# lmb-freiburg/hand3d

Measured on NVIDIA H100. Metric: images/sec full pipeline 320x320, higher is better.
Workload: dtype bf16 hi/lo split x3 MMA passes, fp32 accumulate (fp32 parity, 1e-3)

## Files before the change

### hand3d_b200/_lib.py

```python
from __future__ import annotations

import ctypes as C
import os

HERE = os.path.dirname(os.path.abspath(__file__))
LIB_PATH = os.path.join(HERE, "libhand3d_b200.so")

OK, EINVAL, ENODEVICE, ECUDA, EWEIGHTS, EWORKSPACE = 0, -1, -2, -3, -4, -5
PREC_FP32_FFMA, PREC_BF16X3, PREC_FP16X3, PREC_FP16, PREC_BF16 = 0, 1, 2, 3, 4
PRECISIONS = {"fp32_ffma": 0, "bf16x3": 1, "fp16x3": 2, "fp16": 3, "bf16": 4, "fp16_f8c": 5}
VARIANTS = {"direct": 0, "bottleneck": 1, "proposed": 2, "local": 3, "local_w_xyz_loss": 3}

_p, _i, _i64, _f = C.c_void_p, C.c_int, C.c_int64, C.c_float

SIGNATURES = {
    "h3d_last_error": (C.c_char_p, []),
    "h3d_version": (_i, []),
    "h3d_device_available": (_i, []),
    "h3d_create": (_i, [C.POINTER(_p), _i]),
    "h3d_destroy": (_i, [_p]),
    "h3d_set_precision": (_i, [_p, _i]),
    "h3d_get_precision": (_i, [_p]),
    "h3d_set_tuning": (_i, [_p, C.c_char_p, _i]),
    "h3d_check_errors": (_i, [_p, C.POINTER(_i)]),
# ... 11 lines not shown
    "h3d_pipeline_forward": (_i, [_p, _p, _p, _i, _i, _i, _i, _p, _p, _p, _p, _p, _p, _p, _p, _p, _p, _p]),
    "h3d_pose2d_forward": (_i, [_p, _p, _i, _i, _i, _p, _p, _p]),
    "h3d_track_state_bytes": (_i64, [_i]),
    "h3d_track_step": (_i, [_p, _p, _p, _i, _i, _i, _i, _i, _f, _f, _p, _p, _p, _p, _p, _p, _p, _p]),
    "h3d_track_update": (_i, [_p, _p, _p, _p, _p, _i, _f, _f, _p, _p]),
    "h3d_conv2d_f32": (_i, [_p, _p, _p, _p, _p, _i, _i, _i, _i, _i, _i, _i, _i, _p]),
    "h3d_conv2d_tc": (_i, [_p, _p, _p, _p, _p, _i, _i, _i, _i, _i, _i, _i, _i, _p]),
    "h3d_conv2d_tc_strided": (_i, [_p, _p, _p, _p, _p, _i, _i, _i, _i, _i, _i, _i, _i, _i, _p]),
    "h3d_pack_conv_weights": (_i, [_p, _p, _p, _i, _i, _i, _i, C.POINTER(_p)]),
    "h3d_free_packed_conv": (_i, [_p, _p]),
    "h3d_conv2d_tc_packed": (_i, [_p, _p, _p, _p, _i, _i, _i, _i, _i, _p]),
    "h3d_conv2d_tc_dev": (_i, [_p, _p, _p, _p, _p, _i, _i, _i, _i, _i, _i, _i, _i, _i, _p]),
    "h3d_conv2d_tc_backward": (_i, [_p, _p, _p, _p, _p, _p, _p, _p, _i, _i, _i, _i, _i, _i, _i, _i, _i, _p]),
    "h3d_conv2d_layer_planes": (_i, [_p, _p, _i, _i, _i, _i, _p, _p, _i, _i, _i, _p, _i, _i, _i, _i, _p, _p, _p, _p, _i, _i, _p, _i, _i, _p]),
    "h3d_conv2d_tc_geometry": (_i, [_i, _i, _i, _i, _i, _i, C.POINTER(_i)]),
    "h3d_conv2d_wgrad_geometry": (_i, [_i, _i, _i, _i, _i, _i, C.POINTER(_i)]),
    "h3d_leaky_relu_f32": (_i, [_p, _p, _p, _i64, _p]),
    "h3d_maxpool2x2_f32": (_i, [_p, _p, _p, _i, _i, _i, _i, _p]),
    "h3d_maxpool2x2_backward_f32": (_i, [_p, _p, _p, _p, _i, _i, _i, _i, _p]),
    "h3d_fully_connected_f32": (_i, [_p, _p, _p, _p, _p, _i, _i, _i, _i, _p]),
    "h3d_resize_bilinear_tf1": (_i, [_p, _p, _p, _i, _i, _i, _i, _i, _i, _p]),
    "h3d_avgpool8": (_i, [_p, _p, _p, _i, _i, _i, _i, _p]),
    "h3d_seg_postprocess": (_i, [_p, _p, _i, _i, _i, _p, _p, _p, _p, _p, _p]),
    "h3d_calc_center_bb": (_i, [_p, _p, _i, _i, _i, _p, _p, _p, _p]),
    "h3d_crop_image_from_xy": (_i, [_p, _p, _p, _p, _p, _i, _i, _i, _i, _i, _p]),
    "h3d_detect_keypoints": (_i, [_p, _p, _i, _i, _i, _i, _p, _p]),
    "h3d_upsample_detect_keypoints": (_i, [_p, _p, _i, _i, _i, _i, _i, _p, _p, _p]),
    "h3d_pack_records": (_i, [_p, _p, _p, _p, _p, _i, _p, _p]),
    "h3d_gather_records_p2p": (_i, [_p, _p, _p, _p, _p, _i, _i, _p, _p, C.c_uint64, _i, _i, C.c_uint32, _i64, _p]),
    "h3d_decode_records": (_i, [_p, _i, _p, _i, _i, _p, _p, _p, _p, _p]),
# ... 72 lines not shown
```

### hand3d_b200/csrc/api.cu

```cuda
#include <array>
#include <cstdarg>
#include <cstring>
#include <functional>
#include <map>
#include <memory>
#include <string>
#include <vector>

#include "common.cuh"
#include "split_fmt.cuh"

namespace h3d {

static thread_local char g_err[1024] = "";
void set_error(const char* fmt, ...) {
    va_list ap;
    va_start(ap, fmt);
    vsnprintf(g_err, sizeof(g_err), fmt, ap);
    va_end(ap);
}
int cuda_fail(cudaError_t e, const char* what, const char* file, int line) {
    set_error("CUDA error %d (%s) at %s:%d: %s", (int)e, cudaGetErrorString(e), file, line, what);
    if (e == cudaErrorNoDevice || e == cudaErrorInsufficientDriver) return H3D_ENODEVICE;
    return H3D_ECUDA;
// ... 1458 lines not shown
        d.partial = wpart; d.dw = dw_hwio; d.err_flag = ctx->err_flag;
        if ((rc = launch_conv_wgrad(d, s))) return rc;
        ctx->launches += 3;
    }
    return H3D_OK;
}

int h3d_conv2d_tc_geometry(int B, int H, int W, int Cout, int pool, int precision, int* out) {
    H3D_REQUIRE(out && B > 0 && H > 0 && W > 0 && Cout > 0, "h3d_conv2d_tc_geometry: bad argument");
    H3D_REQUIRE(pool >= 0 && pool <= 2, "h3d_conv2d_tc_geometry: pool must be 0 (none), 1 (max-pool) or 2 (stride 2)");
    H3D_REQUIRE(precision >= H3D_PREC_BF16X3 && precision <= H3D_PREC_FP16_F8C, "h3d_conv2d_tc_geometry: precision must be a tensor-core mode");
    tc_conv_geometry(B, H, W, (int)align_up(Cout, 64), pool, passes_of(precision), out);
    return H3D_OK;
}

int h3d_conv2d_wgrad_geometry(int B, int H, int W, int ksize, int Cin, int Cout, int* out) {
    H3D_REQUIRE(out && B > 0 && H > 0 && W > 0 && Cin > 0 && Cout > 0, "h3d_conv2d_wgrad_geometry: bad argument");
    H3D_REQUIRE(ksize == 1 || ksize == 3 || ksize == 5 || ksize == 7, "h3d_conv2d_wgrad_geometry: ksize must be 1, 3, 5 or 7");
    conv_wgrad_geometry(B, H, W, ksize, (int)align_up(Cin, 64), (int)align_up(Cout, 64), out);
    return H3D_OK;
}

int h3d_conv2d_tc(h3d_ctx* ctx, const float* x, const float* host_w_hwio, const float* host_bias, float* y, int B, int H, int W,
                  int Cin, int Cout, int ksize, int leaky, int precision, void* stream) {
    return h3d_conv2d_tc_strided(ctx, x, host_w_hwio, host_bias, y, B, H, W, Cin, Cout, ksize, 1, leaky, precision, stream);
}

int h3d_conv2d_tc_strided(h3d_ctx* ctx, const float* x, const float* host_w_hwio, const float* host_bias, float* y, int B, int H, int W,
                          int Cin, int Cout, int ksize, int stride, int leaky, int precision, void* stream) {
    H3D_REQUIRE(ctx != nullptr, "ctx is NULL");
// ... 524 lines not shown
```

### hand3d_b200/csrc/common.cuh

```cuda
#pragma once
#include <cuda_runtime.h>
#include <cuda_bf16.h>
#include <cuda_fp16.h>
#include <stdint.h>
#include <stdio.h>
#include <algorithm>
#include <cmath>
#include <string>

#include "../../include/hand3d_b200.h"

namespace h3d {

void set_error(const char* fmt, ...);
int cuda_fail(cudaError_t e, const char* what, const char* file, int line);

#define H3D_CUDA(expr)                                                     \
    do {                                                                   \
        cudaError_t _e = (expr);                                           \
        if (_e != cudaSuccess) return h3d::cuda_fail(_e, #expr, __FILE__, __LINE__); \
    } while (0)

#define H3D_CHECK_LAUNCH() H3D_CUDA(cudaGetLastError())

// ... 167 lines not shown
    int Cout, Cout_pad;
    Split y;
    int Cy_total, cy_off;
    float* yf;
    int Cyf_total, cyf_off;
    int B, H, W, k, leaky;
    int passes;
    float corr_scale = 0.f;
    Half16 half;
    int pool = 0;
    int* err_flag = nullptr;
};
struct TcTuning {
    int bn = 0;
    int chunk_kb = 0;
    int no_side_stream = 0, no_pool_fusion = 0, lift_direct = 0;
    int c3_ffma = 0;
    int no_seg_fusion = 0;
    int fc_chain = 1;
    int pdl = 1;
};
TcTuning& tc_tuning();
int tc_set_tuning(const char* key, int value);
struct FcLayerDesc {
    Split x; int x_stride, in_features;
    Split w; const float* bias; int out_features, out_pad;
    const float* w_scale = nullptr;
    Split y; int y_stride;
    float* yf; int yf_stride;
    int leaky;
};
struct FcChainDesc { FcLayerDesc layer[4]; int num_layers = 0; };
struct FcChainPlan;
FcChainPlan* fc_chain_plan_create(const FcChainDesc* chains, int num_chains, int B, Half16 half, const float* can, const float* uxyz,
                                  unsigned int* counter, int* err_flag);
void fc_chain_plan_destroy(FcChainPlan* p);
int fc_chain_launch(const FcChainPlan* p, const float* hand_side, float* rot, float* out, cudaStream_t s);
TcConvPlan* tc_conv_plan_create(const TcConvDesc& d, int* rc = nullptr);
void tc_conv_plan_destroy(TcConvPlan* p);
int tc_conv_launch(const TcConvPlan* p, cudaStream_t s);
int64_t tc_conv_flops(const TcConvPlan* p);
int tc_num_sms();
void tc_conv_geometry(int B, int H, int W, int Cout_pad, int pool, int passes, int out[4]);

int launch_pack_conv_w(const float* w_hwio, const float* bias, Split out, float* bias_pad, float* w_scale, int k, int Cin, int Cout,
                       int Cin_pad, int Cout_pad, bool dgrad, Half16 half, cudaStream_t s);
int conv_grad_prep_blocks(int64_t pixels, int64_t* pixels_per_block);
int launch_conv_grad_prep(const float* dy, const float* y, Split out, float* db_part, int B, int H, int W, int Cout, int Cout_pad,
                          int stride, int leaky, cudaStream_t s);
int launch_bias_grad_reduce(const float* db_part, int nblk, int Cout, int Cout_pad, float* db, cudaStream_t s);
struct WgradDesc {
    Split x;
    Split dy;
    int B, H, W, Cin, Cout, Cin_pad, Cout_pad, k, passes;
    float* partial;
    float* dw;
    int* err_flag;
};
// ... 28 lines not shown
```

### hand3d_b200/csrc/conv_wgmma.cu

```cuda
#include <cuda.h>

#include <algorithm>
#include <cstdlib>
#include <cstring>
#include <vector>

#include "common.cuh"
#include "split_fmt.cuh"
#include "wgmma_common.cuh"

namespace h3d {

namespace {

constexpr int BM = 128;
constexpr int BK = 64;
constexpr int kThreads = 384;
constexpr int kConsumerThreads = 256;
constexpr int A_TILE_BYTES = BM * BK * 2;
constexpr int STG_COLS = 64;
constexpr int STG_PITCH = STG_COLS + 1;
constexpr int STG_BYTES = BM * STG_PITCH * 4;
constexpr int kSmemBudget = 227 * 1024 - 2048 - STG_BYTES;

__host__ __device__ constexpr int stage_bytes(int BN, int PASSES) { return (PASSES >= 3 ? 2 : 1) * (A_TILE_BYTES + BN * BK * 2); }
__host__ __device__ constexpr int num_stages(int BN, int PASSES) {
    return kSmemBudget / stage_bytes(BN, PASSES) > 8 ? 8 : kSmemBudget / stage_bytes(BN, PASSES);
}
__host__ __device__ constexpr int smem_bytes(int BN, int PASSES) { return num_stages(BN, PASSES) * stage_bytes(BN, PASSES) + STG_BYTES + 2048; }

struct TcParams {
    const float* bias;
    uint16_t* y_hi; uint16_t* y_lo; uint8_t* y_l8; uint8_t* y_h8; int Cy_total, cy_off;
    float corr_scale;
    float* yf; int Cyf_total, cyf_off;
    int B, H, W, k, pad, cin_chunks;
    int TW, TH, TB, tiles_w, tiles_h, n_tiles, num_tiles;
    int n_valid;
    int pool;
    int chunk_kb;
    int leaky;
    int* err_flag;
    const float* w_scale;
};

template <int PASSES, bool FP16, bool SMEM_SCALE = false>
__device__ __forceinline__ void epilogue_store32(const TcParams& p, const float* a, int64_t pix, int n, bool valid, const float* w_scale) {
    float f[32];
    const float4* bp = reinterpret_cast<const float4*>(p.bias + n);
#pragma unroll
    for (int q = 0; q < 8; ++q) {
        const float4 bv = __ldg(bp + q);
        if (PASSES == 4) {
            f[4 * q + 0] = fmaf(a[4 * q + 0], p.corr_scale, bv.x);
            f[4 * q + 1] = fmaf(a[4 * q + 1], p.corr_scale, bv.y);
// ... 185 lines not shown
        fence_regs<NR8>(acc8);
        if constexpr (PASSES == 4) {
#pragma unroll
            for (int i = 0; i < NR; ++i) acc[i] += acc8[i];
        }
        if (kb0 == 0) {
#pragma unroll
            for (int i = 0; i < NR; ++i) racc[i] = acc[i];
        } else {
#pragma unroll
            for (int i = 0; i < NR; ++i) racc[i] += acc[i];
        }
    }
}

template <int BN, int PASSES, bool FP16, class PixOf, bool SMEM_SCALE = false>
__device__ __forceinline__ void store_tile(const TcParams& p, const float* racc, float* stg, int ct, int n0, PixOf pix_of,
                                           const float* w_scale) {
    const int wg = ct >> 7, tt = ct & 127;
    const int r0 = wg * 64 + (tt >> 5) * 16 + ((tt & 31) >> 2);
    const int cq = 2 * (tt & 3);
    const int row = ct & 127, half = ct >> 7;
    int64_t pix; bool valid;
    pix_of(row, pix, valid);
#pragma unroll
    for (int rnd = 0; rnd < BN / STG_COLS; ++rnd) {
        named_bar_sync(1, kConsumerThreads);
#pragma unroll
        for (int j = 0; j < STG_COLS / 8; ++j) {
            const int jj = rnd * (STG_COLS / 8) + j, c = 8 * j + cq;
            stg[r0 * STG_PITCH + c] = racc[4 * jj];
            stg[r0 * STG_PITCH + c + 1] = racc[4 * jj + 1];
            stg[(r0 + 8) * STG_PITCH + c] = racc[4 * jj + 2];
            stg[(r0 + 8) * STG_PITCH + c + 1] = racc[4 * jj + 3];
        }
        named_bar_sync(1, kConsumerThreads);
        float f[32];
#pragma unroll
        for (int q = 0; q < 32; ++q) f[q] = stg[row * STG_PITCH + half * 32 + q];
        epilogue_store32<PASSES, FP16, SMEM_SCALE>(p, f, pix, n0 + rnd * STG_COLS + half * 32, valid, w_scale);
    }
}

constexpr int kProducerRegs = 40, kConsumerRegs = 232;

template <int BN, int PASSES, bool FP16>
__global__ void __launch_bounds__(kThreads, 1)
conv_tc_kernel(const __grid_constant__ CUtensorMap map_x_hi, const __grid_constant__ CUtensorMap map_x_lo,
               const __grid_constant__ CUtensorMap map_w_hi, const __grid_constant__ CUtensorMap map_w_lo,
               const __grid_constant__ CUtensorMap map_x_h8, const __grid_constant__ CUtensorMap map_w_l8, const TcParams p) {
    using C = RingCfg<BN, PASSES>;
    static_assert(PASSES != 4 || FP16, "fp8-correction mode uses an fp16 main plane");
    static_assert(smem_bytes(BN, PASSES) <= 227 * 1024, "conv_tc_kernel: shared memory budget");

    extern __shared__ __align__(1024) uint8_t smem_raw[];
    uint8_t* smem = reinterpret_cast<uint8_t*>((reinterpret_cast<uintptr_t>(smem_raw) + 1023) & ~(uintptr_t)1023);
    float* stg = reinterpret_cast<float*>(smem + C::STAGES * C::STAGE_BYTES);
    uint64_t* bars = reinterpret_cast<uint64_t*>(smem + C::STAGES * C::STAGE_BYTES + STG_BYTES);
    Ring ring{smem, bars, bars + C::STAGES, 0, 0};

    const int warp = threadIdx.x >> 5, lane = threadIdx.x & 31;
    const int wg = __shfl_sync(0xFFFFFFFFu, (int)threadIdx.x / 128, 0);
    const int kblocks = p.k * p.k * p.cin_chunks;

    if (threadIdx.x == 0) {
        prefetch_tmap(&map_x_hi); prefetch_tmap(&map_w_hi);
        if (PASSES >= 3) { prefetch_tmap(&map_x_lo); prefetch_tmap(&map_w_lo); }
        if (PASSES == 4) { prefetch_tmap(&map_x_h8); prefetch_tmap(&map_w_l8); }
        for (int s = 0; s < C::STAGES; ++s) { mbar_init(&ring.full[s], 1); mbar_init(&ring.empty[s], kConsumerThreads / 32); }
        asm volatile("fence.mbarrier_init.release.cluster;" ::: "memory");
    }
    __syncthreads();
    pdl_launch_dependents();
    pdl_wait();

    if (wg == 0) {
        setmaxnreg_dec<kProducerRegs>();
        if (warp == 0) {
            for (int tile = blockIdx.x; tile < p.num_tiles; tile += gridDim.x) {
                const int nt = tile % p.n_tiles, mt = tile / p.n_tiles;
                const int tw = mt % p.tiles_w, th = (mt / p.tiles_w) % p.tiles_h, tb = mt / (p.tiles_w * p.tiles_h);
                const int w0 = tw * p.TW - p.pad, h0 = th * p.TH - p.pad, b0 = tb * p.TB, n0 = nt * BN;
                int kcol = 0;
                for (int kh = 0; kh < p.k; ++kh)
                    for (int kw = 0; kw < p.k; ++kw)
                        for (int cc = 0; cc < p.cin_chunks; ++cc, kcol += BK)
                            produce_kblock<BN, PASSES>(ring, &map_x_hi, &map_x_lo, &map_x_h8, &map_w_hi, &map_w_lo, &map_w_l8, cc * BK,
                                                       w0 + kw, h0 + kh, b0, kcol, n0, p.err_flag);
            }
        }
    } else {
        setmaxnreg_inc<kConsumerRegs>();
        const int ct = threadIdx.x - 128;
        float racc[BN / 2];
        for (int tile = blockIdx.x; tile < p.num_tiles; tile += gridDim.x) {
            const int nt = tile % p.n_tiles, mt = tile / p.n_tiles;
            const int tw = mt % p.tiles_w, th = (mt / p.tiles_w) % p.tiles_h, tb = mt / (p.tiles_w * p.tiles_h);
            mma_tile<BN, PASSES, FP16>(ring, kblocks, p.chunk_kb, racc, ct >> 7, lane, p.err_flag);
            store_tile<BN, PASSES, FP16>(p, racc, stg, ct, nt * BN, [&](int row, int64_t& pix, bool& valid) {
                const int w_l = row % p.TW, h_l = (row / p.TW) % p.TH, b_l = row / (p.TW * p.TH);
                const int w = tw * p.TW + w_l, h = th * p.TH + h_l, b = tb * p.TB + b_l;
                valid = (w < p.W) && (h < p.H) && (b < p.B);
                pix = ((int64_t)b * p.H + h) * p.W + w;
                if (p.pool) {
                    const int par = p.pool == 2 ? 1 : 0;
                    valid = valid && ((w & 1) == par) && ((h & 1) == par);
                    pix = ((int64_t)b * (p.H >> 1) + (h >> 1)) * (p.W >> 1) + (w >> 1);
                }
            }, p.w_scale);
        }
    }
}

constexpr int C3_TW = 16, C3_TH = 8;
constexpr int C3T_THREADS = 256;
constexpr int C3T_B_BYTES = 128 * BK * 2;
constexpr int C3T_PW = C3_TW + 2, C3T_PH = C3_TH + 2;
constexpr int C3T_PATCH_FLOATS = C3T_PH * C3T_PW * 3;
constexpr int C3T_SMEM = C3T_B_BYTES + 2 * A_TILE_BYTES + STG_BYTES + C3T_PATCH_FLOATS * 4 + 64 * 4 + 1024 ;

template <bool FP16>
__global__ void __launch_bounds__(C3T_THREADS, 2)
conv_c3_tc_kernel(const float* __restrict__ x, const float* __restrict__ w, const TcParams p) {
// ... 263 lines not shown
        const int64_t tiles = (int64_t)ceil_div(W, c[0]) * ceil_div(H, c[1]) * ceil_div(B, c[2]);
        if (best < 0 || tiles < best) { best = tiles; *TW = c[0]; *TH = c[1]; *TB = c[2]; }
    }
}

template <int BN, int PASSES, bool FP16>
int launch_inst(const TcConvPlan* pl, cudaStream_t s);

}

struct TcConvPlan {
    int device = 0;
    TcConvDesc d;
    CUtensorMap map_x_hi, map_x_lo, map_w_hi, map_w_lo, map_x_h8, map_w_l8;
    TcParams p;
    int BN, grid;
};

constexpr int kMaxDevices = 64;
static int current_device() { int dev = 0; if (cudaGetDevice(&dev) != cudaSuccess) { cudaGetLastError(); dev = 0; } return dev; }
int tc_num_sms() {
    static int n[kMaxDevices] = {};
    const int dev = current_device() % kMaxDevices;
    if (!n[dev]) {
        int v = 0;
        if (cudaDeviceGetAttribute(&v, cudaDevAttrMultiProcessorCount, dev) != cudaSuccess || v <= 0) { cudaGetLastError(); v = 132; }
        n[dev] = v;
    }
    return n[dev];
}
template <typename K>
// ... 11 lines not shown
    cudaLaunchConfig_t cfg = {};
    cfg.gridDim = grid; cfg.blockDim = block; cfg.dynamicSmemBytes = smem; cfg.stream = s;
    cudaLaunchAttribute attr[1];
    attr[0].id = cudaLaunchAttributeProgrammaticStreamSerialization;
    attr[0].val.programmaticStreamSerializationAllowed = tc_tuning().pdl ? 1 : 0;
    cfg.attrs = attr; cfg.numAttrs = 1;
    return cudaLaunchKernelEx(&cfg, kernel, static_cast<KArgs>(args)...);
}

TcTuning& tc_tuning() {
    static TcTuning t = [] {
        TcTuning v;
        auto geti = [](const char* n, int d) { const char* e = getenv(n); return e ? atoi(e) : d; };
        v.bn = geti("H3D_TC_BN", 0);
        v.chunk_kb = geti("H3D_TC_CHUNK_KB", 0);
        v.no_side_stream = geti("H3D_NO_SIDE_STREAM", 0);
        v.no_pool_fusion = geti("H3D_NO_POOL_FUSION", 0);
        v.lift_direct = geti("H3D_LIFT_DIRECT", 0);
        v.c3_ffma = geti("H3D_C3_FFMA", 0);
        v.pdl = geti("H3D_PDL", 1);
        v.fc_chain = geti("H3D_FC_CHAIN", 1);
        v.no_seg_fusion = geti("H3D_NO_SEG_FUSION", 0);
        return v;
    }();
    return t;
}
int tc_set_tuning(const char* key, int value) {
    TcTuning& t = tc_tuning();
    const std::string k(key ? key : "");
    if (k == "tc_bn") t.bn = value;
    else if (k == "tc_chunk_kb") t.chunk_kb = value;
    else if (k == "no_side_stream") t.no_side_stream = value;
    else if (k == "no_pool_fusion") t.no_pool_fusion = value;
    else if (k == "lift_direct") t.lift_direct = value;
    else if (k == "c3_ffma") t.c3_ffma = value;
    else if (k == "pdl") t.pdl = value;
    else if (k == "fc_chain") t.fc_chain = value;
    else if (k == "no_seg_fusion") t.no_seg_fusion = value;
    else { set_error("h3d_set_tuning: unknown key '%s'", k.c_str()); return H3D_EINVAL; }
    return H3D_OK;
}

namespace {
int choose_bn(int H, int W, int Cout_pad, int passes) {
    const TcTuning& tune = tc_tuning();
    int BN = Cout_pad % 128 == 0 ? 128 : 64;
    if ((int64_t)H * W <= 256) BN = 64;
    if ((tune.bn == 64 || tune.bn == 128) && Cout_pad % tune.bn == 0) BN = tune.bn;
    if (passes == 4) BN = 64;
    return BN;
}

template <int BN, int PASSES, bool FP16>
int launch_inst(const TcConvPlan* pl, cudaStream_t s) {
    constexpr int smem = smem_bytes(BN, PASSES);
    static bool attr[kMaxDevices] = {};
    if (int rc = smem_opt_in(conv_tc_kernel<BN, PASSES, FP16>, smem, attr)) return rc;
    H3D_CUDA(launch_pdl(conv_tc_kernel<BN, PASSES, FP16>, dim3(pl->grid), dim3(kThreads), smem, s, pl->map_x_hi, pl->map_x_lo, pl->map_w_hi,
                        pl->map_w_lo, pl->map_x_h8, pl->map_w_l8, pl->p));
    return H3D_OK;
}
}

TcConvPlan* tc_conv_plan_create(const TcConvDesc& d, int* rc) {
    int rc_local;
    if (!rc) rc = &rc_local;
    *rc = H3D_EINVAL;
    if (d.Cin_pad % BK != 0 || d.Cout_pad % 64 != 0 || (d.k != 1 && d.k != 3 && d.k != 5 && d.k != 7) || (d.passes != 1 && d.passes != 3 && d.passes != 4)) {
        set_error("tc_conv: unsupported geometry (Cin_pad=%d Cout_pad=%d k=%d passes=%d)", d.Cin_pad, d.Cout_pad, d.k, d.passes);
        return nullptr;
    }
    const bool padded_out = d.Cout % 32 != 0;
    if (d.y.hi && ((d.Cy_total % 8) || (d.cy_off % 8))) { set_error("tc_conv: split output channel offset/stride must be multiples of 8"); return nullptr; }
    if (d.yf && !padded_out && ((d.Cyf_total % 4) || (d.cyf_off % 4))) { set_error("tc_conv: fp32 output channel offset/stride must be multiples of 4"); return nullptr; }
// ... 23 lines not shown
    p.y_hi = d.y.hi; p.y_lo = d.y.lo; p.y_l8 = d.y.l8; p.y_h8 = d.y.h8; p.Cy_total = d.Cy_total; p.cy_off = d.cy_off;
    p.corr_scale = d.corr_scale;
    p.yf = d.yf; p.Cyf_total = d.Cyf_total; p.cyf_off = d.cyf_off;
    p.B = d.B; p.H = d.H; p.W = d.W; p.k = d.k; p.pad = d.k / 2; p.cin_chunks = d.Cin_pad / BK;
    p.TW = TW; p.TH = TH; p.TB = TB;
    p.tiles_w = ceil_div(d.W, TW); p.tiles_h = ceil_div(d.H, TH);
    p.n_tiles = d.Cout_pad / BN;
    p.num_tiles = p.tiles_w * p.tiles_h * ceil_div(d.B, TB) * p.n_tiles;
    p.leaky = d.leaky;
    p.n_valid = d.Cout;
    p.pool = d.pool;
    p.err_flag = d.err_flag;
    p.w_scale = d.w_scale;
    p.chunk_kb = d.passes >= 3 ? 9 : 27;
    if (tune.chunk_kb > 0) p.chunk_kb = tune.chunk_kb;
    pl->grid = std::min(p.num_tiles, tc_num_sms());
    const int Ktot = d.k * d.k * d.Cin_pad;
    bool ok = encode_act_map(&pl->map_x_hi, d.x.hi, d.Cin_total, d.Cin_pad, d.W, d.H, d.B, TW, TH, TB) &&
              encode_w_map(&pl->map_w_hi, d.w.hi, Ktot, d.Cout_pad, BN);
    if (ok && d.passes == 3)
        ok = encode_act_map(&pl->map_x_lo, d.x.lo, d.Cin_total, d.Cin_pad, d.W, d.H, d.B, TW, TH, TB) &&
             encode_w_map(&pl->map_w_lo, d.w.lo, Ktot, d.Cout_pad, BN);
    if (ok && d.passes == 4)
        ok = encode_act_map(&pl->map_x_lo, d.x.l8, d.Cin_total, d.Cin_pad, d.W, d.H, d.B, TW, TH, TB, 1) &&
             encode_act_map(&pl->map_x_h8, d.x.h8, d.Cin_total, d.Cin_pad, d.W, d.H, d.B, TW, TH, TB, 1) &&
             encode_w_map(&pl->map_w_lo, d.w.h8, Ktot, d.Cout_pad, BN, 1) &&
             encode_w_map(&pl->map_w_l8, d.w.l8, Ktot, d.Cout_pad, BN, 1);
    if (ok && d.passes == 1) { pl->map_x_lo = pl->map_x_hi; pl->map_w_lo = pl->map_w_hi; }
    if (ok && d.passes != 4) { pl->map_x_h8 = pl->map_x_hi; pl->map_w_l8 = pl->map_w_hi; }
    if (!ok) { delete pl; return nullptr; }
    *rc = H3D_OK;
    return pl;
}

void tc_conv_plan_destroy(TcConvPlan* p) { delete p; }

void tc_conv_geometry(int B, int H, int W, int Cout_pad, int pool, int passes, int out[4]) {
    choose_tile(B, H, W, &out[0], &out[1], &out[2], pool == 1);
    out[3] = choose_bn(H, W, Cout_pad, passes);
}

int64_t tc_conv_flops(const TcConvPlan* p) {
    return 2ll * p->d.B * p->d.H * p->d.W * p->d.k * p->d.k * (int64_t)p->d.Cin_pad * p->d.Cout_pad;
}

int tc_conv_launch(const TcConvPlan* pl, cudaStream_t s) {
    const bool fp16 = pl->d.half == Half16::FP16;
    const int key = pl->BN * 10 + pl->d.passes;
#define CASE(BN_, P_)                                                                  \
    case BN_ * 10 + P_:                                                                \
        return fp16 ? launch_inst<BN_, P_, true>(pl, s) : launch_inst<BN_, P_, false>(pl, s);
    switch (key) {
        CASE(64, 1) CASE(64, 3) CASE(128, 1) CASE(128, 3)
        case 64 * 10 + 4: return launch_inst<64, 4, true>(pl, s);
// ... 84 lines not shown
```

### hand3d_b200/runtime.py

```python
from __future__ import annotations

import ctypes as C

import numpy as np
import torch

from . import _lib
from ._lib import PRECISIONS, VARIANTS


def _ptr(t):
    return C.c_void_p(0 if t is None else t.data_ptr())


def _stream():
    return C.c_void_p(torch.cuda.current_stream().cuda_stream)


def _chk_f32(t, name, ndim=None):
    if not isinstance(t, torch.Tensor):
        raise TypeError("%s must be a torch.Tensor" % name)
    if not t.is_cuda:
        raise RuntimeError("%s must live on a CUDA device (hand3d_b200 has no CPU path)" % name)
    if t.dtype != torch.float32:
# ... 869 lines not shown
        self.reset()

    def reset(self):
        self.center.fill_(160.0)
        self.scale.fill_(float(np.float32(256.0) / (np.float32(100.0) * np.float32(1.25))))
        self.score.fill_(float("nan"))
        self.lost.fill_(1)


def conv2d_tc_geometry(B, H, W, Cout, pool=0, precision="bf16x3"):
    out = (C.c_int * 4)()
    _lib.check(_lib.load().h3d_conv2d_tc_geometry(B, H, W, Cout, int(pool), PRECISIONS[precision], out), "h3d_conv2d_tc_geometry")
    return tuple(out)


def conv2d_wgrad_geometry(B, H, W, ksize, Cin, Cout):
    out = (C.c_int * 6)()
    _lib.check(_lib.load().h3d_conv2d_wgrad_geometry(B, H, W, ksize, Cin, Cout, out), "h3d_conv2d_wgrad_geometry")
    return tuple(out)


_default = {}


def default_context(device=None) -> Context:
    idx = torch.cuda.current_device() if device is None else torch.device(device).index or 0
    if idx not in _default:
        _default[idx] = Context(idx)
    return _default[idx]

# ... 4 lines not shown
```

### include/hand3d_b200.h

```cpp
#ifndef HAND3D_B200_H_
#define HAND3D_B200_H_

#include <stddef.h>
#include <stdint.h>

#if defined(__GNUC__)
#define H3D_API __attribute__((visibility("default")))
#else
#define H3D_API
#endif

#ifdef __cplusplus
extern "C" {
#endif

#define H3D_OK 0
#define H3D_EINVAL (-1)
#define H3D_ENODEVICE (-2)
#define H3D_ECUDA (-3)
#define H3D_EWEIGHTS (-4)
#define H3D_EWORKSPACE (-5)

#define H3D_PREC_FP32_FFMA 0
#define H3D_PREC_BF16X3 1
// ... 71 lines not shown
H3D_API int h3d_pack_conv_weights(h3d_ctx* ctx, const float* host_w_hwio, const float* host_bias, int ksize, int Cin, int Cout,
                                  int precision, h3d_packed_conv** out);
H3D_API int h3d_free_packed_conv(h3d_ctx* ctx, h3d_packed_conv* packed);
H3D_API int h3d_conv2d_tc_packed(h3d_ctx* ctx, const float* x, const h3d_packed_conv* packed, float* y, int B, int H, int W,
                                 int stride, int leaky, void* stream);
H3D_API int h3d_conv2d_tc_dev(h3d_ctx* ctx, const float* x, const float* w_hwio, const float* bias, float* y, int B, int H, int W,
                              int Cin, int Cout, int ksize, int stride, int leaky, int precision, void* stream);
H3D_API int h3d_conv2d_layer_planes(h3d_ctx* ctx, const float* x, int B, int H, int W, int Cx, const float* host_w_hwio,
                                    const float* host_bias, int ksize, int Cin, int Cout, const int32_t* host_perm, int pool, int leaky,
                                    int precision, int route, void* y_hi, void* y_lo, void* y_l8, void* y_h8, int Cy_total, int cy_off,
                                    float* yf, int Cyf_total, int cyf_off, void* stream);
H3D_API int h3d_conv2d_tc_backward(h3d_ctx* ctx, const float* x, const float* y, const float* dy, const float* w_hwio, float* dx,
                                   float* dw_hwio, float* db, int B, int H, int W, int Cin, int Cout, int ksize, int stride, int leaky,
                                   int precision, void* stream);
H3D_API int h3d_conv2d_tc_geometry(int B, int H, int W, int Cout, int pool, int precision, int* out);
H3D_API int h3d_conv2d_wgrad_geometry(int B, int H, int W, int ksize, int Cin, int Cout, int* out);
H3D_API int h3d_leaky_relu_f32(h3d_ctx* ctx, const float* x, float* y, int64_t n, void* stream);
H3D_API int h3d_maxpool2x2_f32(h3d_ctx* ctx, const float* x, float* y, int B, int H, int W, int C, void* stream);
H3D_API int h3d_maxpool2x2_backward_f32(h3d_ctx* ctx, const float* x, const float* dy, float* dx, int B, int H, int W, int C, void* stream);
H3D_API int h3d_fully_connected_f32(h3d_ctx* ctx, const float* x, const float* w, const float* bias, float* y,
                            int B, int in_features, int out_features, int leaky, void* stream);
H3D_API int h3d_resize_bilinear_tf1(h3d_ctx* ctx, const float* x, float* y, int B, int H, int W, int C,
                            int out_h, int out_w, void* stream);
H3D_API int h3d_avgpool8(h3d_ctx* ctx, const float* x, float* y, int B, int H, int W, int C, void* stream);
H3D_API int h3d_seg_postprocess(h3d_ctx* ctx, const float* logits, int B, int H, int W, uint8_t* hand_mask,
                        int32_t* max_loc, float* center, float* crop_size, float* scale_crop, void* stream);
H3D_API int h3d_calc_center_bb(h3d_ctx* ctx, const float* mask, int B, int H, int W, float* center, float* bb, float* crop_size,
                               void* stream);
H3D_API int h3d_crop_image_from_xy(h3d_ctx* ctx, const float* image, const float* center, const float* scale,
                           float* image_crop, int B, int H, int W, int C, int crop_size, void* stream);
// ... 132 lines not shown
```

Baseline: 1243.

## Reuse activation row tiles across kernel rows in bf16x3 wgmma conv

For the 3-pass tensor-core conv, the producer now loads a taller activation box (TH+run-1 rows) once per (kw, cin chunk) and reuses it across several kh taps by offsetting the smem descriptor by TW rows. Separate A and B rings with their own mbarriers replace the single combined stage ring. The K loop is reordered to kw/cc/kh to make this possible. The aim is to cut redundant TMA activation traffic per k×k kernel. The cost is fewer pipeline stages for A, more shared memory per A slot, and a more complex synchronisation scheme.

```diff
diff --git a/hand3d_b200/_lib.py b/hand3d_b200/_lib.py
--- a/hand3d_b200/_lib.py
+++ b/hand3d_b200/_lib.py
@@ -49,6 +49,7 @@
     "h3d_conv2d_tc_backward": (_i, [_p, _p, _p, _p, _p, _p, _p, _p, _i, _i, _i, _i, _i, _i, _i, _i, _i, _p]),
     "h3d_conv2d_layer_planes": (_i, [_p, _p, _i, _i, _i, _i, _p, _p, _i, _i, _i, _p, _i, _i, _i, _i, _p, _p, _p, _p, _i, _i, _p, _i, _i, _p]),
     "h3d_conv2d_tc_geometry": (_i, [_i, _i, _i, _i, _i, _i, C.POINTER(_i)]),
+    "h3d_conv2d_tc_row_run": (_i, [_i, _i, _i, _i, _i, _i, _i, _i, C.POINTER(_i)]),
     "h3d_conv2d_wgrad_geometry": (_i, [_i, _i, _i, _i, _i, _i, C.POINTER(_i)]),
     "h3d_leaky_relu_f32": (_i, [_p, _p, _p, _i64, _p]),
     "h3d_maxpool2x2_f32": (_i, [_p, _p, _p, _i, _i, _i, _i, _p]),
diff --git a/hand3d_b200/csrc/api.cu b/hand3d_b200/csrc/api.cu
--- a/hand3d_b200/csrc/api.cu
+++ b/hand3d_b200/csrc/api.cu
@@ -1496,6 +1496,15 @@
     return H3D_OK;
 }
 
+int h3d_conv2d_tc_row_run(int B, int H, int W, int Cin, int Cout, int ksize, int pool, int precision, int* out) {
+    H3D_REQUIRE(out && B > 0 && H > 0 && W > 0 && Cin > 0 && Cout > 0, "h3d_conv2d_tc_row_run: bad argument");
+    H3D_REQUIRE(ksize == 1 || ksize == 3 || ksize == 5 || ksize == 7, "h3d_conv2d_tc_row_run: ksize must be 1, 3, 5 or 7");
+    H3D_REQUIRE(pool >= 0 && pool <= 2, "h3d_conv2d_tc_row_run: pool must be 0 (none), 1 (max-pool) or 2 (stride 2)");
+    H3D_REQUIRE(precision >= H3D_PREC_BF16X3 && precision <= H3D_PREC_FP16_F8C, "h3d_conv2d_tc_row_run: precision must be a tensor-core mode");
+    tc_conv_row_run(B, H, W, (int)align_up(Cout, 64), ksize, pool, passes_of(precision), out);
+    return H3D_OK;
+}
+
 int h3d_conv2d_wgrad_geometry(int B, int H, int W, int ksize, int Cin, int Cout, int* out) {
     H3D_REQUIRE(out && B > 0 && H > 0 && W > 0 && Cin > 0 && Cout > 0, "h3d_conv2d_wgrad_geometry: bad argument");
     H3D_REQUIRE(ksize == 1 || ksize == 3 || ksize == 5 || ksize == 7, "h3d_conv2d_wgrad_geometry: ksize must be 1, 3, 5 or 7");
diff --git a/hand3d_b200/csrc/common.cuh b/hand3d_b200/csrc/common.cuh
--- a/hand3d_b200/csrc/common.cuh
+++ b/hand3d_b200/csrc/common.cuh
@@ -205,6 +205,7 @@
 struct TcTuning {
     int bn = 0;
     int chunk_kb = 0;
+    int row_reuse = 1;
     int no_side_stream = 0, no_pool_fusion = 0, lift_direct = 0;
     int c3_ffma = 0;
     int no_seg_fusion = 0;
@@ -233,6 +234,7 @@
 int64_t tc_conv_flops(const TcConvPlan* p);
 int tc_num_sms();
 void tc_conv_geometry(int B, int H, int W, int Cout_pad, int pool, int passes, int out[4]);
+void tc_conv_row_run(int B, int H, int W, int Cout_pad, int k, int pool, int passes, int out[2]);
 
 int launch_pack_conv_w(const float* w_hwio, const float* bias, Split out, float* bias_pad, float* w_scale, int k, int Cin, int Cout,
                        int Cin_pad, int Cout_pad, bool dgrad, Half16 half, cudaStream_t s);
diff --git a/hand3d_b200/csrc/conv_wgmma.cu b/hand3d_b200/csrc/conv_wgmma.cu
--- a/hand3d_b200/csrc/conv_wgmma.cu
+++ b/hand3d_b200/csrc/conv_wgmma.cu
@@ -23,11 +23,14 @@
 constexpr int STG_BYTES = BM * STG_PITCH * 4;
 constexpr int kSmemBudget = 227 * 1024 - 2048 - STG_BYTES;
 
-__host__ __device__ constexpr int stage_bytes(int BN, int PASSES) { return (PASSES >= 3 ? 2 : 1) * (A_TILE_BYTES + BN * BK * 2); }
+__host__ __device__ constexpr int a_slot_bytes(int rows, int PASSES) { return (PASSES >= 3 ? 2 : 1) * rows * BK * 2; }
+__host__ __device__ constexpr int b_slot_bytes(int BN, int PASSES) { return (PASSES >= 3 ? 2 : 1) * BN * BK * 2; }
+__host__ __device__ constexpr int stage_bytes(int BN, int PASSES) { return a_slot_bytes(BM, PASSES) + b_slot_bytes(BN, PASSES); }
 __host__ __device__ constexpr int num_stages(int BN, int PASSES) {
     return kSmemBudget / stage_bytes(BN, PASSES) > 8 ? 8 : kSmemBudget / stage_bytes(BN, PASSES);
 }
 __host__ __device__ constexpr int smem_bytes(int BN, int PASSES) { return num_stages(BN, PASSES) * stage_bytes(BN, PASSES) + STG_BYTES + 2048; }
+constexpr int kMaxSmemBytes = kSmemBudget + STG_BYTES + 2048;
 
 struct TcParams {
     const float* bias;
@@ -39,6 +42,7 @@
     int n_valid;
     int pool;
     int chunk_kb;
+    int run, a_wg_rows, a_slot, a_slots, b_slots;
     int leaky;
     int* err_flag;
     const float* w_scale;
@@ -254,6 +258,120 @@
     }
 }
 
+struct Rings {
+    uint8_t* a; uint8_t* b;
+    uint64_t *a_full, *a_empty, *b_full, *b_empty;
+    int a_slot, a_slots, b_slots;
+    int a_stage, b_stage;
+    uint32_t a_phase, b_phase;
+};
+
+__device__ __forceinline__ float* rings_init(Rings& r, uint8_t* smem, int a_slot, int a_slots, int b_slot, int b_slots) {
+    r.a = smem; r.b = smem + a_slots * a_slot;
+    float* stg = reinterpret_cast<float*>(r.b + b_slots * b_slot);
+    uint64_t* bars = reinterpret_cast<uint64_t*>(reinterpret_cast<uint8_t*>(stg) + STG_BYTES);
+    r.a_full = bars; r.a_empty = bars + a_slots; r.b_full = bars + 2 * a_slots; r.b_empty = bars + 2 * a_slots + b_slots;
+    r.a_slot = a_slot; r.a_slots = a_slots; r.b_slots = b_slots;
+    r.a_stage = r.b_stage = 0; r.a_phase = r.b_phase = 0;
+    if (threadIdx.x == 0) {
+        for (int s = 0; s < a_slots; ++s) { mbar_init(&r.a_full[s], 1); mbar_init(&r.a_empty[s], kConsumerThreads / 32); }
+        for (int s = 0; s < b_slots; ++s) { mbar_init(&r.b_full[s], 1); mbar_init(&r.b_empty[s], kConsumerThreads / 32); }
+    }
+    return stg;
+}
+
+__device__ __forceinline__ void produce_a(Rings& r, const CUtensorMap* x_hi, const CUtensorMap* x_lo, int a0, int a1, int a2, int a3,
+                                          int* err_flag) {
+    mbar_wait(&r.a_empty[r.a_stage], r.a_phase ^ 1, err_flag, 1);
+    if (elect_one()) {
+        uint8_t* st = r.a + r.a_stage * r.a_slot;
+        uint64_t* fb = &r.a_full[r.a_stage];
+        mbar_expect_tx(fb, r.a_slot);
+        tma_load_4d(x_hi, st, fb, a0, a1, a2, a3);
+        tma_load_4d(x_lo, st + r.a_slot / 2, fb, a0, a1, a2, a3);
+    }
+    __syncwarp();
+    if (++r.a_stage == r.a_slots) { r.a_stage = 0; r.a_phase ^= 1; }
+}
+
+template <int BN>
+__device__ __forceinline__ void produce_b(Rings& r, const CUtensorMap* w_hi, const CUtensorMap* w_lo, int kcol, int n0, int* err_flag) {
+    constexpr int SLOT = b_slot_bytes(BN, 3);
+    mbar_wait(&r.b_empty[r.b_stage], r.b_phase ^ 1, err_flag, 1);
+    if (elect_one()) {
+        uint8_t* st = r.b + r.b_stage * SLOT;
+        uint64_t* fb = &r.b_full[r.b_stage];
+        mbar_expect_tx(fb, SLOT);
+        tma_load_2d(w_hi, st, fb, kcol, n0);
+        tma_load_2d(w_lo, st + SLOT / 2, fb, kcol, n0);
+    }
+    __syncwarp();
+    if (++r.b_stage == r.b_slots) { r.b_stage = 0; r.b_phase ^= 1; }
+}
+
+template <int BN, bool FP16>
+__device__ __forceinline__ void mma_tile_runs(Rings& r, int kblocks, int k, int run, int a_wg_rows, int row_step, int chunk_kb,
+                                              float* racc, int wg, int lane, int* err_flag) {
+    constexpr int NR = BN / 2;
+    constexpr int B_PLANE = BN * BK * 2;
+    float acc[NR];
+#pragma unroll
+    for (int i = 0; i < NR; ++i) acc[i] = 0.f;
+    const int a_plane = r.a_slot / 2;
+    int kh = 0, kh0 = 0;
+    for (int kb0 = 0; kb0 < kblocks; kb0 += chunk_kb) {
+        const int kb1 = min(kblocks, kb0 + chunk_kb);
+        int pend_b = -1, pend_a = -1;
+        for (int kb = kb0; kb < kb1; ++kb) {
+            if (kh == kh0) mbar_wait(&r.a_full[r.a_stage], r.a_phase, err_flag, 3);
+            mbar_wait(&r.b_full[r.b_stage], r.b_phase, err_flag, 3);
+            const int a_row = wg * a_wg_rows + (kh - kh0) * row_step;
+            const uint32_t sa = smem_u32(r.a + r.a_stage * r.a_slot) + a_row * 128;
+            const uint32_t sb = smem_u32(r.b + r.b_stage * b_slot_bytes(BN, 3));
+            const uint64_t a_hi = desc_sw128(sa), a_lo = desc_sw128(sa + a_plane);
+            const uint64_t b_hi = desc_sw128(sb), b_lo = desc_sw128(sb + B_PLANE);
+            fence_regs<NR>(acc);
+            wgmma_fence();
+#pragma unroll
+            for (int j = 0; j < BK / 16; ++j) {
+                const uint64_t koff = (uint64_t)j * 2;
+                mma16<BN, FP16>(acc, a_hi + koff, b_hi + koff, (uint32_t)((kb > kb0) | (j != 0)));
+                mma16<BN, FP16>(acc, a_hi + koff, b_lo + koff, 1u);
+                mma16<BN, FP16>(acc, a_lo + koff, b_hi + koff, 1u);
+            }
+            wgmma_commit();
+            fence_regs<NR>(acc);
+            wgmma_wait<1>();
+            if (pend_b >= 0 && lane == 0) {
+                mbar_arrive(&r.b_empty[pend_b]);
+                if (pend_a >= 0) mbar_arrive(&r.a_empty[pend_a]);
+            }
+            pend_b = r.b_stage;
+            if (++r.b_stage == r.b_slots) { r.b_stage = 0; r.b_phase ^= 1; }
+            const bool run_end = kh + 1 == k || kh + 1 - kh0 == run;
+            pend_a = run_end ? r.a_stage : -1;
+            if (++kh == k) kh = 0;
+            if (run_end) {
+                kh0 = kh;
+                if (++r.a_stage == r.a_slots) { r.a_stage = 0; r.a_phase ^= 1; }
+            }
+        }
+        wgmma_wait<0>();
+        if (lane == 0) {
+            mbar_arrive(&r.b_empty[pend_b]);
+            if (pend_a >= 0) mbar_arrive(&r.a_empty[pend_a]);
+        }
+        fence_regs<NR>(acc);
+        if (kb0 == 0) {
+#pragma unroll
+            for (int i = 0; i < NR; ++i) racc[i] = acc[i];
+        } else {
+#pragma unroll
+            for (int i = 0; i < NR; ++i) racc[i] += acc[i];
+        }
+    }
+}
+
 template <int BN, int PASSES, bool FP16, class PixOf, bool SMEM_SCALE = false>
 __device__ __forceinline__ void store_tile(const TcParams& p, const float* racc, float* stg, int ct, int n0, PixOf pix_of,
                                            const float* w_scale) {
@@ -284,6 +402,62 @@
 
 constexpr int kProducerRegs = 40, kConsumerRegs = 232;
 
+__device__ __forceinline__ void conv_pix_of(const TcParams& p, int tw, int th, int tb, int row, int64_t& pix, bool& valid) {
+    const int w_l = row % p.TW, h_l = (row / p.TW) % p.TH, b_l = row / (p.TW * p.TH);
+    const int w = tw * p.TW + w_l, h = th * p.TH + h_l, b = tb * p.TB + b_l;
+    valid = (w < p.W) && (h < p.H) && (b < p.B);
+    pix = ((int64_t)b * p.H + h) * p.W + w;
+    if (p.pool) {
+        const int par = p.pool == 2 ? 1 : 0;
+        valid = valid && ((w & 1) == par) && ((h & 1) == par);
+        pix = ((int64_t)b * (p.H >> 1) + (h >> 1)) * (p.W >> 1) + (w >> 1);
+    }
+}
+
+template <int BN, bool FP16>
+__device__ __forceinline__ void conv_row_runs(const CUtensorMap& map_x_hi, const CUtensorMap& map_x_lo, const CUtensorMap& map_w_hi,
+                                              const CUtensorMap& map_w_lo, const TcParams& p, uint8_t* smem) {
+    Rings ring;
+    float* stg = rings_init(ring, smem, p.a_slot, p.a_slots, b_slot_bytes(BN, 3), p.b_slots);
+    if (threadIdx.x == 0) asm volatile("fence.mbarrier_init.release.cluster;" ::: "memory");
+    __syncthreads();
+    pdl_launch_dependents();
+    pdl_wait();
+
+    const int warp = threadIdx.x >> 5, lane = threadIdx.x & 31;
+    const int wg = __shfl_sync(0xFFFFFFFFu, (int)threadIdx.x / 128, 0);
+    if (wg == 0) {
+        setmaxnreg_dec<kProducerRegs>();
+        if (warp == 0) {
+            for (int tile = blockIdx.x; tile < p.num_tiles; tile += gridDim.x) {
+                const int nt = tile % p.n_tiles, mt = tile / p.n_tiles;
+                const int tw = mt % p.tiles_w, th = (mt / p.tiles_w) % p.tiles_h, tb = mt / (p.tiles_w * p.tiles_h);
+                const int w0 = tw * p.TW - p.pad, h0 = th * p.TH - p.pad, b0 = tb * p.TB, n0 = nt * BN;
+                for (int kw = 0; kw < p.k; ++kw)
+                    for (int cc = 0; cc < p.cin_chunks; ++cc)
+                        for (int kh0 = 0; kh0 < p.k; kh0 += p.run) {
+                            produce_a(ring, &map_x_hi, &map_x_lo, cc * BK, w0 + kw, h0 + kh0, b0, p.err_flag);
+                            for (int kh = kh0; kh < min(p.k, kh0 + p.run); ++kh)
+                                produce_b<BN>(ring, &map_w_hi, &map_w_lo, ((kh * p.k + kw) * p.cin_chunks + cc) * BK, n0, p.err_flag);
+                        }
+            }
+        }
+    } else {
+        setmaxnreg_inc<kConsumerRegs>();
+        const int ct = threadIdx.x - 128;
+        float racc[BN / 2];
+        for (int tile = blockIdx.x; tile < p.num_tiles; tile += gridDim.x) {
+            const int nt = tile % p.n_tiles, mt = tile / p.n_tiles;
+            const int tw = mt % p.tiles_w, th = (mt / p.tiles_w) % p.tiles_h, tb = mt / (p.tiles_w * p.tiles_h);
+            mma_tile_runs<BN, FP16>(ring, p.k * p.k * p.cin_chunks, p.k, p.run, p.a_wg_rows, p.TW, p.chunk_kb, racc, ct >> 7, lane,
+                                    p.err_flag);
+            store_tile<BN, 3, FP16>(p, racc, stg, ct, nt * BN, [&](int row, int64_t& pix, bool& valid) {
+                conv_pix_of(p, tw, th, tb, row, pix, valid);
+            }, p.w_scale);
+        }
+    }
+}
+
 template <int BN, int PASSES, bool FP16>
 __global__ void __launch_bounds__(kThreads, 1)
 conv_tc_kernel(const __grid_constant__ CUtensorMap map_x_hi, const __grid_constant__ CUtensorMap map_x_lo,
@@ -295,18 +469,26 @@
 
     extern __shared__ __align__(1024) uint8_t smem_raw[];
     uint8_t* smem = reinterpret_cast<uint8_t*>((reinterpret_cast<uintptr_t>(smem_raw) + 1023) & ~(uintptr_t)1023);
-    float* stg = reinterpret_cast<float*>(smem + C::STAGES * C::STAGE_BYTES);
-    uint64_t* bars = reinterpret_cast<uint64_t*>(smem + C::STAGES * C::STAGE_BYTES + STG_BYTES);
-    Ring ring{smem, bars, bars + C::STAGES, 0, 0};
-
-    const int warp = threadIdx.x >> 5, lane = threadIdx.x & 31;
-    const int wg = __shfl_sync(0xFFFFFFFFu, (int)threadIdx.x / 128, 0);
-    const int kblocks = p.k * p.k * p.cin_chunks;
-
     if (threadIdx.x == 0) {
         prefetch_tmap(&map_x_hi); prefetch_tmap(&map_w_hi);
         if (PASSES >= 3) { prefetch_tmap(&map_x_lo); prefetch_tmap(&map_w_lo); }
         if (PASSES == 4) { prefetch_tmap(&map_x_h8); prefetch_tmap(&map_w_l8); }
+    }
+    if constexpr (PASSES == 3) {
+        if (p.run > 1) {
+            conv_row_runs<BN, FP16>(map_x_hi, map_x_lo, map_w_hi, map_w_lo, p, smem);
+            return;
+        }
+    }
+    float* stg = reinterpret_cast<float*>(smem + C::STAGES * C::STAGE_BYTES);
+    uint64_t* bars = reinterpret_cast<uint64_t*>(smem + C::STAGES * C::STAGE_BYTES + STG_BYTES);
+    Ring ring{smem, bars, bars + C::STAGES, 0, 0};
+
+    const int warp = threadIdx.x >> 5, lane = threadIdx.x & 31;
+    const int wg = __shfl_sync(0xFFFFFFFFu, (int)threadIdx.x / 128, 0);
+    const int kblocks = p.k * p.k * p.cin_chunks;
+
+    if (threadIdx.x == 0) {
         for (int s = 0; s < C::STAGES; ++s) { mbar_init(&ring.full[s], 1); mbar_init(&ring.empty[s], kConsumerThreads / 32); }
         asm volatile("fence.mbarrier_init.release.cluster;" ::: "memory");
     }
@@ -321,12 +503,21 @@
                 const int nt = tile % p.n_tiles, mt = tile / p.n_tiles;
                 const int tw = mt % p.tiles_w, th = (mt / p.tiles_w) % p.tiles_h, tb = mt / (p.tiles_w * p.tiles_h);
                 const int w0 = tw * p.TW - p.pad, h0 = th * p.TH - p.pad, b0 = tb * p.TB, n0 = nt * BN;
-                int kcol = 0;
-                for (int kh = 0; kh < p.k; ++kh)
+                if constexpr (PASSES == 3) {
                     for (int kw = 0; kw < p.k; ++kw)
-                        for (int cc = 0; cc < p.cin_chunks; ++cc, kcol += BK)
-                            produce_kblock<BN, PASSES>(ring, &map_x_hi, &map_x_lo, &map_x_h8, &map_w_hi, &map_w_lo, &map_w_l8, cc * BK,
-                                                       w0 + kw, h0 + kh, b0, kcol, n0, p.err_flag);
+                        for (int cc = 0; cc < p.cin_chunks; ++cc)
+                            for (int kh = 0; kh < p.k; ++kh)
+                                produce_kblock<BN, PASSES>(ring, &map_x_hi, &map_x_lo, &map_x_h8, &map_w_hi, &map_w_lo, &map_w_l8, cc * BK,
+                                                           w0 + kw, h0 + kh, b0, ((kh * p.k + kw) * p.cin_chunks + cc) * BK, n0,
+                                                           p.err_flag);
+                } else {
+                    int kcol = 0;
+                    for (int kh = 0; kh < p.k; ++kh)
+                        for (int kw = 0; kw < p.k; ++kw)
+                            for (int cc = 0; cc < p.cin_chunks; ++cc, kcol += BK)
+                                produce_kblock<BN, PASSES>(ring, &map_x_hi, &map_x_lo, &map_x_h8, &map_w_hi, &map_w_lo, &map_w_l8, cc * BK,
+                                                           w0 + kw, h0 + kh, b0, kcol, n0, p.err_flag);
+                }
             }
         }
     } else {
@@ -338,15 +529,7 @@
             const int tw = mt % p.tiles_w, th = (mt / p.tiles_w) % p.tiles_h, tb = mt / (p.tiles_w * p.tiles_h);
             mma_tile<BN, PASSES, FP16>(ring, kblocks, p.chunk_kb, racc, ct >> 7, lane, p.err_flag);
             store_tile<BN, PASSES, FP16>(p, racc, stg, ct, nt * BN, [&](int row, int64_t& pix, bool& valid) {
-                const int w_l = row % p.TW, h_l = (row / p.TW) % p.TH, b_l = row / (p.TW * p.TH);
-                const int w = tw * p.TW + w_l, h = th * p.TH + h_l, b = tb * p.TB + b_l;
-                valid = (w < p.W) && (h < p.H) && (b < p.B);
-                pix = ((int64_t)b * p.H + h) * p.W + w;
-                if (p.pool) {
-                    const int par = p.pool == 2 ? 1 : 0;
-                    valid = valid && ((w & 1) == par) && ((h & 1) == par);
-                    pix = ((int64_t)b * (p.H >> 1) + (h >> 1)) * (p.W >> 1) + (w >> 1);
-                }
+                conv_pix_of(p, tw, th, tb, row, pix, valid);
             }, p.w_scale);
         }
     }
@@ -640,7 +823,7 @@
     TcConvDesc d;
     CUtensorMap map_x_hi, map_x_lo, map_w_hi, map_w_lo, map_x_h8, map_w_l8;
     TcParams p;
-    int BN, grid;
+    int BN, grid, smem;
 };
 
 constexpr int kMaxDevices = 64;
@@ -682,6 +865,7 @@
         auto geti = [](const char* n, int d) { const char* e = getenv(n); return e ? atoi(e) : d; };
         v.bn = geti("H3D_TC_BN", 0);
         v.chunk_kb = geti("H3D_TC_CHUNK_KB", 0);
+        v.row_reuse = geti("H3D_TC_ROW_REUSE", 1);
         v.no_side_stream = geti("H3D_NO_SIDE_STREAM", 0);
         v.no_pool_fusion = geti("H3D_NO_POOL_FUSION", 0);
         v.lift_direct = geti("H3D_LIFT_DIRECT", 0);
@@ -698,6 +882,7 @@
     const std::string k(key ? key : "");
     if (k == "tc_bn") t.bn = value;
     else if (k == "tc_chunk_kb") t.chunk_kb = value;
+    else if (k == "tc_row_reuse") t.row_reuse = value;
     else if (k == "no_side_stream") t.no_side_stream = value;
     else if (k == "no_pool_fusion") t.no_pool_fusion = value;
     else if (k == "lift_direct") t.lift_direct = value;
@@ -719,13 +904,19 @@
     return BN;
 }
 
+int row_run(int k, int passes, int BN, int TW, int TH, int TB) {
+    if (!tc_tuning().row_reuse || k == 1 || passes != 3 || TW % 8 != 0 || !(TB == 1 || (TB == 2 && TW * TH == 64))) return 0;
+    int rmax = 1;
+    while (rmax < k && 2 * a_slot_bytes(TW * (TH + rmax) * TB, passes) + 3 * b_slot_bytes(BN, passes) <= kSmemBudget) ++rmax;
+    return ceil_div(k, ceil_div(k, rmax));
+}
+
 template <int BN, int PASSES, bool FP16>
 int launch_inst(const TcConvPlan* pl, cudaStream_t s) {
-    constexpr int smem = smem_bytes(BN, PASSES);
     static bool attr[kMaxDevices] = {};
-    if (int rc = smem_opt_in(conv_tc_kernel<BN, PASSES, FP16>, smem, attr)) return rc;
-    H3D_CUDA(launch_pdl(conv_tc_kernel<BN, PASSES, FP16>, dim3(pl->grid), dim3(kThreads), smem, s, pl->map_x_hi, pl->map_x_lo, pl->map_w_hi,
-                        pl->map_w_lo, pl->map_x_h8, pl->map_w_l8, pl->p));
+    if (int rc = smem_opt_in(conv_tc_kernel<BN, PASSES, FP16>, kMaxSmemBytes, attr)) return rc;
+    H3D_CUDA(launch_pdl(conv_tc_kernel<BN, PASSES, FP16>, dim3(pl->grid), dim3(kThreads), (size_t)pl->smem, s, pl->map_x_hi, pl->map_x_lo,
+                        pl->map_w_hi, pl->map_w_lo, pl->map_x_h8, pl->map_w_l8, pl->p));
     return H3D_OK;
 }
 }
@@ -779,12 +970,23 @@
     p.w_scale = d.w_scale;
     p.chunk_kb = d.passes >= 3 ? 9 : 27;
     if (tune.chunk_kb > 0) p.chunk_kb = tune.chunk_kb;
+    p.run = std::max(1, row_run(d.k, d.passes, BN, TW, TH, TB));
+    const int box_h = TH + p.run - 1;
+    if (p.run > 1) {
+        p.a_wg_rows = TB == 1 ? 64 : TW * box_h;
+        p.a_slot = a_slot_bytes(TW * box_h * TB, d.passes);
+        p.a_slots = 2;
+        p.b_slots = std::min(8, (kSmemBudget - p.a_slots * p.a_slot) / b_slot_bytes(BN, d.passes));
+        pl->smem = p.a_slots * p.a_slot + p.b_slots * b_slot_bytes(BN, d.passes) + STG_BYTES + 2048;
+    } else {
+        pl->smem = smem_bytes(BN, d.passes);
+    }
     pl->grid = std::min(p.num_tiles, tc_num_sms());
     const int Ktot = d.k * d.k * d.Cin_pad;
-    bool ok = encode_act_map(&pl->map_x_hi, d.x.hi, d.Cin_total, d.Cin_pad, d.W, d.H, d.B, TW, TH, TB) &&
+    bool ok = encode_act_map(&pl->map_x_hi, d.x.hi, d.Cin_total, d.Cin_pad, d.W, d.H, d.B, TW, box_h, TB) &&
               encode_w_map(&pl->map_w_hi, d.w.hi, Ktot, d.Cout_pad, BN);
     if (ok && d.passes == 3)
-        ok = encode_act_map(&pl->map_x_lo, d.x.lo, d.Cin_total, d.Cin_pad, d.W, d.H, d.B, TW, TH, TB) &&
+        ok = encode_act_map(&pl->map_x_lo, d.x.lo, d.Cin_total, d.Cin_pad, d.W, d.H, d.B, TW, box_h, TB) &&
              encode_w_map(&pl->map_w_lo, d.w.lo, Ktot, d.Cout_pad, BN);
     if (ok && d.passes == 4)
         ok = encode_act_map(&pl->map_x_lo, d.x.l8, d.Cin_total, d.Cin_pad, d.W, d.H, d.B, TW, TH, TB, 1) &&
@@ -803,6 +1005,14 @@
 void tc_conv_geometry(int B, int H, int W, int Cout_pad, int pool, int passes, int out[4]) {
     choose_tile(B, H, W, &out[0], &out[1], &out[2], pool == 1);
     out[3] = choose_bn(H, W, Cout_pad, passes);
+}
+
+void tc_conv_row_run(int B, int H, int W, int Cout_pad, int k, int pool, int passes, int out[2]) {
+    int g[4];
+    tc_conv_geometry(B, H, W, Cout_pad, pool, passes, g);
+    const int run = row_run(k, passes, g[3], g[0], g[1], g[2]);
+    out[0] = run > 0;
+    out[1] = std::max(1, run);
 }
 
 int64_t tc_conv_flops(const TcConvPlan* p) {
diff --git a/hand3d_b200/runtime.py b/hand3d_b200/runtime.py
--- a/hand3d_b200/runtime.py
+++ b/hand3d_b200/runtime.py
@@ -907,6 +907,13 @@
     return tuple(out)
 
 
+def conv2d_tc_row_run(B, H, W, Cin, Cout, ksize, pool=0, precision="bf16x3"):
+    out = (C.c_int * 2)()
+    _lib.check(_lib.load().h3d_conv2d_tc_row_run(B, H, W, Cin, Cout, ksize, int(pool), PRECISIONS[precision], out),
+               "h3d_conv2d_tc_row_run")
+    return tuple(out)
+
+
 def conv2d_wgrad_geometry(B, H, W, ksize, Cin, Cout):
     out = (C.c_int * 6)()
     _lib.check(_lib.load().h3d_conv2d_wgrad_geometry(B, H, W, ksize, Cin, Cout, out), "h3d_conv2d_wgrad_geometry")
diff --git a/include/hand3d_b200.h b/include/hand3d_b200.h
--- a/include/hand3d_b200.h
+++ b/include/hand3d_b200.h
@@ -109,6 +109,7 @@
                                    float* dw_hwio, float* db, int B, int H, int W, int Cin, int Cout, int ksize, int stride, int leaky,
                                    int precision, void* stream);
 H3D_API int h3d_conv2d_tc_geometry(int B, int H, int W, int Cout, int pool, int precision, int* out);
+H3D_API int h3d_conv2d_tc_row_run(int B, int H, int W, int Cin, int Cout, int ksize, int pool, int precision, int* out);
 H3D_API int h3d_conv2d_wgrad_geometry(int B, int H, int W, int ksize, int Cin, int Cout, int* out);
 H3D_API int h3d_leaky_relu_f32(h3d_ctx* ctx, const float* x, float* y, int64_t n, void* stream);
 H3D_API int h3d_maxpool2x2_f32(h3d_ctx* ctx, const float* x, float* y, int B, int H, int W, int C, void* stream);
```

New measurement: 1279, median of 6. 1.03x the previous value.
